# OpenDriveLab/OccNet

Measured on AMD Instinct MI355X. Metric: nuScenes samples/sec (6-cam 900x1600 -> 200x200x16 voxels), higher is better.
Workload: dtype f32 hot path (GEMM operands bf16x3-split, SCA value rows q16 block floating point) + bf16 backbone

## Files before the change

### include/occnet_amd.h

```cpp
#ifndef OCCNET_AMD_H_
#define OCCNET_AMD_H_

#include <stdint.h>

#ifdef __cplusplus
extern "C" {
#endif

#define OCC_OK 0
#define OCC_E_INVALID (-1)
#define OCC_E_LAUNCH (-2)
#define OCC_E_UNSUPPORTED (-3)

int occ_abi_version(void);
const char* occ_last_error(void);
int occ_selftest_fdiv_f32(const float* a, const float* d, float* q, int64_t n, void* stream);


int occ_ms_deform_attn_forward_f32(const float* value, const int64_t* spatial_shapes,
                                   const int64_t* level_start_index, const float* sampling_loc,
                                   const float* attn_weight, float* out, int B, int S, int M, int D,
                                   int L, int Lq, int P, int im2col_step, void* stream);

int occ_ms_deform_attn_backward_f32(const float* value, const int64_t* spatial_shapes,
// ... 113 lines not shown

int occ_sca_prep_forward_f32(const float* proj, int64_t proj_batch_stride, int proj_ld, const int64_t* row_to_query,
                             const float* ref_rb, const int64_t* spatial_shapes, float* loc, float* attn, int B,
                             int64_t R, int M, int L, int P, int Z, void* stream);
int occ_sca_prep_backward_f32(const float* grad_loc, const float* grad_attn, const float* attn,
                              const int64_t* query_to_rows, int Kq, const int64_t* spatial_shapes, float* dproj,
                              int proj_ld, int B, int64_t R, int64_t Q, int M, int L, int P, void* stream);

int occ_rows_gather_sum_f32(const float* x, int64_t x_batch_stride, const int64_t* index, int K, float* out, int B,
                            int64_t rows_out, int64_t rows_in, int F, void* stream);

int64_t occ_linear_wgrad_workspace_bytes(int M, int N, int K);
int occ_linear_wgrad_bf16x3_f32(const float* dy, int64_t lddy, const float* x, int64_t ldx, float* dw, float* db,
                                void* workspace, int64_t workspace_bytes, int M, int N, int K, void* stream);

int64_t occ_conv3d_wgrad_workspace_bytes(int B, int Z, int Y, int X, int Cin);
int occ_conv3d_wgrad_bf16x3_f32(const float* dy_pad, const float* x_pad, float* dw, void* workspace,
                                int64_t workspace_bytes, int B, int Z, int Y, int X, int Cin, void* stream);

int occ_bias_act_nhwc_bf16(void* x, const float* bias, const void* residual, int64_t rows, int C, int relu,
                           void* stream);

int64_t occ_bias_act_bwd_partial_floats(int64_t rows, int C);
int occ_bias_act_bwd_nhwc_bf16(const void* grad_y, const void* y, void* g, float* partial, float* bias_grad,
                               int64_t rows, int C, int relu, void* stream);

int occ_conv_bn_fold_fwd_f32(const float* weight, const float* gamma, const float* beta, const float* rstd,
                             const float* mean_rstd, float* w_folded, void* w_folded_bf16_nhwc, float* bias, int Cout,
                             int Cin, int KH, int KW, void* stream);
int occ_conv_bn_fold_bwd_f32(const void* grad_w_bf16, int64_t stride_o, int64_t stride_i, int64_t stride_h, int64_t stride_w,
                             const float* weight, const float* gamma, const float* rstd, const float* mean_rstd,
                             const float* grad_bias, float* grad_weight, float* grad_gamma, int Cout, int Cin, int KH, int KW,
                             void* stream);

unsigned occ_ln_dropout_hash(unsigned index, unsigned seed_lo, unsigned seed_hi);
int64_t occ_dropout_add_ln_bwd_partial_floats(int64_t rows, int C);
int occ_dropout_add_ln_fwd_f32(const float* x, const float* residual, const float* gamma, const float* beta, float eps,
                               float p_drop, uint64_t seed, float* z, float* y, float* stats, int64_t rows, int C,
                               void* stream);
int occ_dropout_add_ln_bwd_f32(const float* grad_y, const float* z, const float* stats, const float* gamma, float p_drop,
                               uint64_t seed, float* grad_x, float* grad_residual, float* partial, float* grad_gamma_beta,
                               int64_t rows, int C, void* stream);

int occ_value_proj_bf16_f32(int n_segments, const void* const* a, const int64_t* lda, const int64_t* rows,
                            const int64_t* rows_per_group, const int64_t* out_row0,
                            const float* const* group_bias, int bias_groups, const void* weight_packed,
                            float* out, int64_t ldo, int K, int N, int64_t out_group_rows, void* stream);
int occ_value_proj_bf16_f16pairs(int n_segments, const void* const* a, const int64_t* lda, const int64_t* rows,
                            const int64_t* rows_per_group, const int64_t* out_row0,
                            const float* const* group_bias, int bias_groups, const void* weight_packed,
                            void* out, int64_t ldo, int K, int N, int64_t out_group_rows, const float* out_scale,
                            void* stream);
int occ_value_proj_bf16_q16pairs(int n_segments, const void* const* a, const int64_t* lda, const int64_t* rows,
                            const int64_t* rows_per_group, const int64_t* out_row0,
                            const float* const* group_bias, int bias_groups, const void* weight_packed,
                            void* out, int64_t ldo, int K, int N, int64_t out_group_rows, const float* out_scale,
                            void* stream);

int occ_value_range_scale_bf16(int n_segments, const void* const* a, const int64_t* lda, const int64_t* rows, int K,
                               int n_planes, const float* row_l1, const float* bias_max, float* scale_out,
                               uint32_t* work, void* stream);
int occ_value_range_scale_from_amax(const uint32_t* amax8, int n_planes, const float* row_l1, const float* bias_max,
                                    float* scale_out, void* stream);

int occ_value_proj_bf16_planes(int n_segments, const void* const* a, const int64_t* lda, const int64_t* rows,
                               const int64_t* rows_per_group, const int64_t* out_row0,
                               const float* const* group_bias, int bias_groups, const void* weight_packed, void* out,
                               int out_f16, int64_t ldo, int K, int n_planes, int plane_cols, int64_t plane_stride,
                               int64_t out_group_rows, const float* out_scale, void* stream);

int occ_stem_conv7x7_pool_f32_bf16(const float* x, const void* weight_frag, const float* bias, void* out,
                                   int batch, int H, int W, void* stream);
int occ_stem_conv7x7_pool_u8_bf16(const uint8_t* x, const void* weight_frag, const float* bias, void* out,
                                  int batch, int Hs, int Ws, int H, int W, const float* mean,
                                  const float* std, int to_rgb, void* stream);

int occ_bias_relu_maxpool_nhwc_bf16(const void* y, const float* bias, void* out, int batch, int H, int W, int C,
                                    void* stream);

int occ_conv1x1_nhwc_bf16(const void* x, const void* weight, const float* bias, const void* residual,
                          void* out, int batch, int Hin, int Win, int Cin, int Cout, int stride, int relu,
                          int residual_upsample2, void* stream);

int occ_conv3x3_pack_weight_bf16(const float* weight, void* packed, int Cout, int Cin, void* stream);
int occ_conv3x3_nhwc_bf16(const void* x, const void* weight_packed, const float* bias, void* out, int batch,
                          int H, int W, int Cin, int Cout, int stride, int relu, void* stream);
int occ_conv3x3_nhwc_bf16_amax(const void* x, const void* weight_packed, const float* bias, void* out, int batch,
                               int H, int W, int Cin, int Cout, int stride, int relu, uint32_t* amax8, void* stream);

int occ_mfma_pack_b_frag_bf16(const float* weight, void* packed, int N, int K, void* stream);

int occ_bottleneck64_nhwc_bf16(const void* x, const void* w1_frag, const float* b1, const void* w2_frag,
                               const float* b2, const void* w3_frag, const float* b3, void* out, int batch,
                               int H, int W, int Cin, int downsample, void* stream);

#ifdef __cplusplus
}
#endif
#endif
```

### occnet_amd/csrc/conv1x1_nhwc_bf16.hip

```cpp
#include "common.h"

namespace occ {

typedef float f32x16 __attribute__((ext_vector_type(16)));
typedef __bf16 bf16x8 __attribute__((ext_vector_type(8)));


__device__ __forceinline__ float c1_bf16_to_f32(unsigned short h) { return __uint_as_float((unsigned)h << 16); }

template <int NT, int RT>
__global__ __launch_bounds__(256) void conv1x1_nhwc_bf16_kernel(
    const uint4* __restrict__ x, const uint4* __restrict__ w, const float* __restrict__ bias,
    const unsigned short* __restrict__ residual, unsigned short* __restrict__ out, long M, int N, int K,
    int Hin, int Win, int Hout, int Wout, int stride, int relu, int res_up) {
  constexpr int KC = 32, kCLD = KC * 2 + 16, PC = KC / 8;
  constexpr int BM = 32 * RT, BN = 128 * NT, WR = 32 * NT, OLD = BN + 4;
  constexpr int AP = BM * PC / 256;
  constexpr int A_BYTES = BM * kCLD;
  constexpr int STAGE_BYTES = 2 * A_BYTES, OUT_BYTES = 32 * OLD * 4;
  __shared__ __attribute__((aligned(16))) char lds[STAGE_BYTES > OUT_BYTES ? STAGE_BYTES : OUT_BYTES];
  const int tid = threadIdx.x, lane = tid & 63, wave = tid >> 6;
  const int vi = lane & 31, kb = lane >> 5;
  const long m0 = (long)blockIdx.x * BM;
  const int n0 = blockIdx.y * BN;
// ... 57 lines not shown
        af[rt][ks] = *reinterpret_cast<const bf16x8*>(sA + (rt * 32 + vi) * kCLD + ks * 32 + kb * 16); \
    _Pragma("unroll") for (int rt = 0; rt < RT; ++rt) {                                           \
      acc[rt][0] = __builtin_amdgcn_mfma_f32_32x32x16_bf16(af[rt][0], __builtin_bit_cast(bf16x8, wa0_##SW), acc[rt][0], 0, 0, 0); \
      if (NT > 1) acc[rt][NT - 1] = __builtin_amdgcn_mfma_f32_32x32x16_bf16(af[rt][0], __builtin_bit_cast(bf16x8, wa1_##SW), acc[rt][NT - 1], 0, 0, 0); \
    }                                                                                             \
    _Pragma("unroll") for (int rt = 0; rt < RT; ++rt) {                                           \
      acc[rt][0] = __builtin_amdgcn_mfma_f32_32x32x16_bf16(af[rt][1], __builtin_bit_cast(bf16x8, wb0_##SW), acc[rt][0], 0, 0, 0); \
      if (NT > 1) acc[rt][NT - 1] = __builtin_amdgcn_mfma_f32_32x32x16_bf16(af[rt][1], __builtin_bit_cast(bf16x8, wb1_##SW), acc[rt][NT - 1], 0, 0, 0); \
    }                                                                                             \
  }

  const int NCHK = K / KC;
  const int rot = (int)((blockIdx.x * 5u + blockIdx.y * 3u) % (unsigned)NCHK);
#define OCC_C1_K(CI) ((((CI) < NCHK ? (CI) : NCHK - 1) + rot) % NCHK * KC)
  OCC_C1_ISSUE_A(0, OCC_C1_K(0))
  OCC_C1_ISSUE_W(0, OCC_C1_K(0))
  OCC_C1_ISSUE_A(1, OCC_C1_K(1))
  OCC_C1_ISSUE_W(1, OCC_C1_K(1))
  for (int ci = 0; ci < NCHK; ci += 6) {
    OCC_C1_STEP(0, 0, 2, 0, OCC_C1_K(ci + 2))
    if (ci + 1 < NCHK) OCC_C1_STEP(1, 1, 0, 1, OCC_C1_K(ci + 3))
    if (ci + 2 < NCHK) OCC_C1_STEP(0, 2, 1, 0, OCC_C1_K(ci + 4))
    if (ci + 3 < NCHK) OCC_C1_STEP(1, 0, 2, 1, OCC_C1_K(ci + 5))
    if (ci + 4 < NCHK) OCC_C1_STEP(0, 1, 0, 0, OCC_C1_K(ci + 6))
    if (ci + 5 < NCHK) OCC_C1_STEP(1, 2, 1, 1, OCC_C1_K(ci + 7))
  }
#undef OCC_C1_K
#undef OCC_C1_STEP
#undef OCC_C1_ISSUE_A
#undef OCC_C1_ISSUE_W

  const int c = lane * 4;
  const bool col_live = c < BN && n0 + c < N;
  float4 bv = make_float4(0.f, 0.f, 0.f, 0.f);
  if (col_live) bv = *reinterpret_cast<const float4*>(bias + n0 + c);
  float* sO = reinterpret_cast<float*>(lds);
#pragma unroll
  for (int rt = 0; rt < RT; ++rt) {
    __syncthreads();
#pragma unroll
    for (int t = 0; t < NT; ++t)
#pragma unroll
      for (int r = 0; r < 16; ++r)
        sO[((r & 3) + 8 * (r >> 2) + 4 * kb) * OLD + (wave * NT + t) * 32 + vi] = acc[rt][t][r];
    __syncthreads();
    uint2 rv[8];
#pragma unroll
    for (int rr = 0; rr < 8; ++rr) {
      long m = m0 + rt * 32 + wave * 8 + rr;
      if (m >= M) m = M - 1;
      rv[rr] = make_uint2(0u, 0u);
      if (residual != nullptr && col_live) {
        long rrow = m;
        if (res_up) {
          const long hw = (long)Hout * Wout;
          const long n = m / hw, rem = m - n * hw;
          const int yo = (int)(rem / Wout), xo = (int)(rem - (long)yo * Wout);
          rrow = (n * (Hout >> 1) + (yo >> 1)) * (Wout >> 1) + (xo >> 1);
        }
        rv[rr] = *reinterpret_cast<const uint2*>(residual + rrow * N + n0 + c);
      }
    }
#pragma unroll
    for (int rr = 0; rr < 8; ++rr) {
      const int row = wave * 8 + rr;
      const long m = m0 + rt * 32 + row;
      if (m < M && col_live) {
        float4 v = *reinterpret_cast<const float4*>(sO + row * OLD + c);
        v.x += bv.x; v.y += bv.y; v.z += bv.z; v.w += bv.w;
        v.x += c1_bf16_to_f32((unsigned short)(rv[rr].x & 0xffffu));
        v.y += c1_bf16_to_f32((unsigned short)(rv[rr].x >> 16));
        v.z += c1_bf16_to_f32((unsigned short)(rv[rr].y & 0xffffu));
        v.w += c1_bf16_to_f32((unsigned short)(rv[rr].y >> 16));
        if (relu) {
          v.x = fmaxf(v.x, 0.f); v.y = fmaxf(v.y, 0.f); v.z = fmaxf(v.z, 0.f); v.w = fmaxf(v.w, 0.f);
        }
        const uint2 o = make_uint2(pack_bf16x2_rne(v.x, v.y), pack_bf16x2_rne(v.z, v.w));
        *reinterpret_cast<uint2*>(out + m * N + n0 + c) = o;
      }
    }
  }
}

}

extern "C" int occ_conv1x1_nhwc_bf16(const void* x, const void* weight, const float* bias,
                                     const void* residual, void* out, int batch, int Hin, int Win,
                                     int Cin, int Cout, int stride, int relu, int residual_upsample2,
                                     void* stream) {
  using namespace occ;
  OCC_CHECK_ARG(x && weight && bias && out, "conv1x1_nhwc_bf16: null pointer argument");
  OCC_CHECK_ARG(batch > 0 && Hin > 0 && Win > 0 && Cin > 0 && Cout > 0 && stride > 0,
                "conv1x1_nhwc_bf16: bad dimension");
  if (Cin % 32 || Cout % 32) {
    set_error("conv1x1_nhwc_bf16: no kernel for Cin=%d Cout=%d (need Cin %% 32 == 0, Cout %% 32 == 0)", Cin,
              Cout);
    return OCC_E_UNSUPPORTED;
  }
  const int Hout = (Hin - 1) / stride + 1, Wout = (Win - 1) / stride + 1;
  OCC_CHECK_ARG(!residual_upsample2 || (residual && Hout % 2 == 0 && Wout % 2 == 0),
                "conv1x1_nhwc_bf16: an upsampled residual needs even output sizes (exact x2 nearest upsampling)");
  const long M = (long)batch * Hout * Wout;
  hipStream_t st = reinterpret_cast<hipStream_t>(stream);
#define OCC_C1_LAUNCH(NTT, RTT, BNN)                                                                \
  hipLaunchKernelGGL((conv1x1_nhwc_bf16_kernel<NTT, RTT>),                                          \
                     dim3((unsigned)((M + 32 * RTT - 1) / (32 * RTT)), (unsigned)((Cout + BNN - 1) / BNN)), \
                     dim3(256), 0, st, reinterpret_cast<const uint4*>(x),                           \
                     reinterpret_cast<const uint4*>(weight), bias,                                  \
                     reinterpret_cast<const unsigned short*>(residual),                             \
                     reinterpret_cast<unsigned short*>(out), M, Cout, Cin, Hin, Win, Hout, Wout, stride, relu,  \
                     residual_upsample2)
  if (Cout <= 128) OCC_C1_LAUNCH(1, 2, 128); else OCC_C1_LAUNCH(2, 2, 256);
#undef OCC_C1_LAUNCH
  OCC_CHECK_LAUNCH("conv1x1_nhwc_bf16");
  return OCC_OK;
}
```

### occnet_amd/ext.py

```python
import ctypes
import os

import torch

from . import _lib, cache_epoch
from ._lib import OccAmdError, OccAmdUnsupported, f32, i32, i64, ptr, stream_ptr


_TIMING = None
_TIMING_ONLY = None


def kernel_timing(enable=True):
    global _TIMING, _TIMING_ONLY
    _TIMING = {} if enable else None
    _TIMING_ONLY = None
    return _TIMING


def kernel_timing_only(names):
    global _TIMING_ONLY
    _TIMING_ONLY = None if names is None else set(names)


# ... 1284 lines not shown
                                                       i32(H), i32(W), stream_ptr(x.device))
    _note_flops('bb_stem7x7_pool', 2.0 * N * Hc * Wc * 64 * 147)
    _lib.check(rc, "stem_conv7x7_pool")
    return out


def stem_conv7x7_pool_u8(x_u8, weight_frag, bias, mean, std, to_rgb=False, size_divisor=32):
    if not (x_u8.is_cuda and x_u8.dtype == torch.uint8 and x_u8.dim() == 4 and x_u8.shape[-1] == 3
            and x_u8.is_contiguous()):
        raise OccAmdUnsupported("stem_conv7x7_pool_u8: x must be a contiguous (N, H, W, 3) uint8 device tensor")
    _need_cuda_f32("bias", bias)
    if weight_frag.numel() != 64 * 224 or bias.numel() != 64:
        raise OccAmdError("stem_conv7x7_pool_u8: inconsistent shapes")
    N, Hs, Ws, _ = x_u8.shape
    d = int(size_divisor)
    H, W = (Hs + d - 1) // d * d, (Ws + d - 1) // d * d
    Hc, Wc = (H - 1) // 2 + 1, (W - 1) // 2 + 1
    Hp, Wp = (Hc - 1) // 2 + 1, (Wc - 1) // 2 + 1
    out = torch.empty((N, 64, Hp, Wp), dtype=torch.bfloat16, device=x_u8.device, memory_format=torch.channels_last)
    mean_c = (f32 * 3)(*[float(v) for v in mean])
    std_c = (f32 * 3)(*[float(v) for v in std])
    with torch.cuda.device(x_u8.device):
        rc = _lib.lib().occ_stem_conv7x7_pool_u8_bf16(ptr(x_u8), ptr(weight_frag), ptr(bias), ptr(out), i32(N),
                                                      i32(Hs), i32(Ws), i32(H), i32(W), mean_c, std_c,
                                                      i32(1 if to_rgb else 0), stream_ptr(x_u8.device))
    _lib.check(rc, "stem_conv7x7_pool_u8")
    return out, (H, W)


def bias_relu_maxpool_nhwc(y, bias):
    if not (y.is_cuda and y.dtype == torch.bfloat16 and y.dim() == 4
            and y.is_contiguous(memory_format=torch.channels_last)):
        raise OccAmdUnsupported("bias_relu_maxpool_nhwc: y must be a channels_last bfloat16 device tensor")
    _need_cuda_f32("bias", bias)
    N, C, H, W = y.shape
    if bias.numel() != C:
        raise OccAmdError("bias_relu_maxpool_nhwc: bias must have C entries")
    out = torch.empty((N, C, (H - 1) // 2 + 1, (W - 1) // 2 + 1), dtype=torch.bfloat16, device=y.device,
                      memory_format=torch.channels_last)
    with torch.cuda.device(y.device):
        rc = _lib.lib().occ_bias_relu_maxpool_nhwc_bf16(ptr(y), ptr(bias), ptr(out), i32(N), i32(H), i32(W),
                                                        i32(C), stream_ptr(y.device))
    _lib.check(rc, "bias_relu_maxpool_nhwc")
    return out


def conv1x1_pack_weight(weight2d):
    cout, cin = weight2d.shape
    if cin % 32 or cout % 32:
        raise OccAmdUnsupported("conv1x1_pack_weight: Cin and Cout must be multiples of 32")
    return mfma_pack_b_frag(weight2d.float().contiguous())


def conv1x1_nhwc(x, weight_frag, bias, residual=None, relu=False, stride=1, residual_upsample2=False):
    if not (x.is_cuda and x.dtype == torch.bfloat16 and x.dim() == 4
            and x.is_contiguous(memory_format=torch.channels_last)):
        raise OccAmdUnsupported("conv1x1_nhwc: x must be a channels_last bfloat16 device tensor")
    _need_cuda_f32("bias", bias)
    N, Cin, H, W = x.shape
    Cout = bias.numel()
    if not (weight_frag.dtype == torch.int16 and weight_frag.dim() == 1 and weight_frag.is_contiguous()
            and weight_frag.numel() == Cout * Cin):
        raise OccAmdError("conv1x1_nhwc: weight must come from conv1x1_pack_weight (Cout*Cin bf16, fragment order)")
    s = int(stride)
    Ho, Wo = (H - 1) // s + 1, (W - 1) // s + 1
    out = torch.empty((N, Cout, Ho, Wo), dtype=torch.bfloat16, device=x.device,
                      memory_format=torch.channels_last)
    want = (N, Cout, Ho // 2, Wo // 2) if residual_upsample2 else tuple(out.shape)
    if residual_upsample2 and (residual is None or Ho % 2 or Wo % 2):
        raise OccAmdUnsupported("conv1x1_nhwc: an upsampled residual needs even output sizes")
    if residual is not None and not (residual.dtype == torch.bfloat16 and tuple(residual.shape) == want and
                                     residual.is_contiguous(memory_format=torch.channels_last)):
        raise OccAmdUnsupported("conv1x1_nhwc: residual must match the output (channels_last bfloat16)")
    with torch.cuda.device(x.device), _timed('bb_conv1x1'):
        rc = _lib.lib().occ_conv1x1_nhwc_bf16(ptr(x), ptr(weight_frag), ptr(bias), ptr(residual), ptr(out),
                                              i32(N), i32(H), i32(W), i32(Cin), i32(Cout), i32(s),
                                              i32(1 if relu else 0), i32(1 if residual_upsample2 else 0),
                                              stream_ptr(x.device))
    _note_flops('bb_conv1x1', 2.0 * N * Ho * Wo * Cin * Cout)
    _lib.check(rc, "conv1x1_nhwc")
    return out


def mfma_pack_b_frag(weight2d):
    _need_cuda_f32("weight", weight2d)
    if weight2d.dim() != 2:
        raise OccAmdError("mfma_pack_b_frag: expected a (N, K) matrix")
    weight2d = weight2d.contiguous()
    n, k = weight2d.shape
    packed = torch.empty(n * k, dtype=torch.int16, device=weight2d.device)
    with torch.cuda.device(weight2d.device):
        rc = _lib.lib().occ_mfma_pack_b_frag_bf16(ptr(weight2d), ptr(packed), i32(n), i32(k),
                                                  stream_ptr(weight2d.device))
    _lib.check(rc, "mfma_pack_b_frag")
    return packed


def bottleneck64_pack(w1, b1, w2, b2, w3, b3, wds=None, bds=None):
    w1 = w1.float().reshape(w1.shape[0], -1)
    w3 = w3.float().reshape(w3.shape[0], -1)
    if tuple(w2.shape) != (64, 64, 3, 3) or w1.shape[0] != 64 or tuple(w3.shape) != (256, 64):
        raise OccAmdUnsupported("bottleneck64_pack: only 64 mid / 256 output channels")
    ds = wds is not None
    cin = w1.shape[1]
    if (ds and cin != 64) or (not ds and cin != 256):
        raise OccAmdUnsupported("bottleneck64_pack: Cin must be 256 (identity) or 64 (projection)")
    w2m = w2.float().permute(0, 2, 3, 1).reshape(64, 9 * 64)
    b3 = b3.float()
    if ds:
        w3 = torch.cat([w3, wds.float().reshape(256, 64)], dim=1)
        b3 = b3 + bds.float()
    return dict(w1=mfma_pack_b_frag(w1), b1=b1.float().contiguous(), w2=mfma_pack_b_frag(w2m),
                b2=b2.float().contiguous(), w3=mfma_pack_b_frag(w3), b3=b3.contiguous(), cin=cin, ds=ds)


def bottleneck64_nhwc(x, pack):
    if not (x.is_cuda and x.dtype == torch.bfloat16 and x.dim() == 4
            and x.is_contiguous(memory_format=torch.channels_last)):
        raise OccAmdUnsupported("bottleneck64_nhwc: x must be a channels_last bfloat16 device tensor")
    N, Cin, H, W = x.shape
    if Cin != pack['cin']:
        raise OccAmdError("bottleneck64_nhwc: x has %d channels, the pack was built for %d" % (Cin, pack['cin']))
    out = torch.empty((N, 256, H, W), dtype=torch.bfloat16, device=x.device, memory_format=torch.channels_last)
    with torch.cuda.device(x.device), _timed('bb_bottleneck64'):
        rc = _lib.lib().occ_bottleneck64_nhwc_bf16(ptr(x), ptr(pack['w1']), ptr(pack['b1']), ptr(pack['w2']),
                                                   ptr(pack['b2']), ptr(pack['w3']), ptr(pack['b3']), ptr(out),
                                                   i32(N), i32(H), i32(W), i32(Cin), i32(1 if pack['ds'] else 0),
                                                   stream_ptr(x.device))
    _note_flops('bb_bottleneck64', 2.0 * N * H * W * (Cin * 64 + 9 * 64 * 64 + 64 * 256 + (Cin * 256 if pack['ds'] else 0)))
    _lib.check(rc, "bottleneck64_nhwc")
    return out


def conv3x3_pack_weight(weight):
    _need_cuda_f32("weight", weight)
    if weight.dim() != 4 or tuple(weight.shape[2:]) != (3, 3):
        raise OccAmdError("conv3x3_pack_weight: expected a (Cout, Cin, 3, 3) weight")
    cout, cin = weight.shape[:2]
    packed = torch.empty(weight.numel(), dtype=torch.int16, device=weight.device)
    with torch.cuda.device(weight.device):
        rc = _lib.lib().occ_conv3x3_pack_weight_bf16(ptr(weight), ptr(packed), i32(cout), i32(cin),
                                                     stream_ptr(weight.device))
    _lib.check(rc, "conv3x3_pack_weight")
    return packed


def conv3x3_nhwc(x, w_packed, bias, cout, relu=False, stride=1, amax=None):
    if not (x.is_cuda and x.dtype == torch.bfloat16 and x.dim() == 4
            and x.is_contiguous(memory_format=torch.channels_last)):
        raise OccAmdUnsupported("conv3x3_nhwc: x must be a channels_last bfloat16 device tensor")
    _need_cuda_f32("bias", bias)
    N, Cin, H, W = x.shape
    if w_packed.numel() != cout * Cin * 9 or bias.numel() != cout:
        raise OccAmdError("conv3x3_nhwc: inconsistent shapes")
    st = int(stride)
    if st not in (1, 2):
        raise OccAmdUnsupported("conv3x3_nhwc: stride must be 1 or 2")
    if amax is not None and not (amax.is_cuda and amax.dtype == torch.int32 and amax.numel() == 8 and amax.is_contiguous()):
        raise OccAmdError("conv3x3_nhwc: amax must be 8 contiguous int32 device words")
    out = torch.empty((N, cout, (H - 1) // st + 1, (W - 1) // st + 1), dtype=torch.bfloat16, device=x.device,
                      memory_format=torch.channels_last)
    with torch.cuda.device(x.device), _timed('bb_conv3x3'):
        if amax is None:
            rc = _lib.lib().occ_conv3x3_nhwc_bf16(ptr(x), ptr(w_packed), ptr(bias), ptr(out), i32(N), i32(H),
                                                  i32(W), i32(Cin), i32(cout), i32(st), i32(1 if relu else 0),
                                                  stream_ptr(x.device))
# ... 8 lines not shown
```

### occnet_amd/plugin/backbone.py

```python
import os

import torch
import torch.nn as nn
import torch.nn.functional as F

from .. import cache_epoch
from .bricks import BaseModule, ConvModule
from .registry import BACKBONES, NECKS


def conv_bn_folded(x, conv, bn):
    rstd, mean_rstd = _bn_fold_constants(bn)
    s = bn.weight * rstd
    w = conv.weight * s.view(-1, 1, 1, 1)
    b = torch.addcmul(bn.bias, bn.weight, mean_rstd, value=-1.0)
    if conv.bias is not None:
        b = b + conv.bias * s
    return F.conv2d(x, w, b, conv.stride, conv.padding, conv.dilation, conv.groups)


def _bn_fold_constants(bn):
    key = (bn.running_mean._version, bn.running_var._version, bn.running_var.data_ptr(), cache_epoch())
    cached = getattr(bn, '_occ_fold', None)
    if cached is None or cached[0] != key:
# ... 249 lines not shown
                if isinstance(m, nn.modules.batchnorm._BatchNorm):
                    m.eval()
        return self


@NECKS.register_module()
class FPN(BaseModule):

    def __init__(self, in_channels, out_channels, num_outs, start_level=0, end_level=-1,
                 add_extra_convs=False, relu_before_extra_convs=False, no_norm_on_lateral=False,
                 conv_cfg=None, norm_cfg=None, act_cfg=None, upsample_cfg=dict(mode='nearest'),
                 init_cfg=None, **kwargs):
        super().__init__(init_cfg)
        assert isinstance(in_channels, (list, tuple))
        self.in_channels, self.out_channels = in_channels, out_channels
        self.num_ins, self.num_outs = len(in_channels), num_outs
        self.relu_before_extra_convs = relu_before_extra_convs
        self.upsample_cfg = dict(upsample_cfg)
        self.backbone_end_level = self.num_ins if end_level in (-1, self.num_ins - 1) else end_level + 1
        self.start_level = start_level
        if add_extra_convs is True:
            add_extra_convs = 'on_input'
        assert add_extra_convs in (False, 'on_input', 'on_lateral', 'on_output')
        self.add_extra_convs = add_extra_convs
        self.lateral_convs = nn.ModuleList()
        self.fpn_convs = nn.ModuleList()
        for i in range(self.start_level, self.backbone_end_level):
            self.lateral_convs.append(ConvModule(in_channels[i], out_channels, 1, conv_cfg=conv_cfg,
                                                 norm_cfg=None if no_norm_on_lateral else norm_cfg,
                                                 act_cfg=act_cfg, inplace=False))
            self.fpn_convs.append(ConvModule(out_channels, out_channels, 3, padding=1,
                                             conv_cfg=conv_cfg, norm_cfg=norm_cfg, act_cfg=act_cfg,
                                             inplace=False))
        extra_levels = num_outs - self.backbone_end_level + self.start_level
        if self.add_extra_convs and extra_levels >= 1:
            for i in range(extra_levels):
                cin = self.in_channels[self.backbone_end_level - 1] \
                    if (i == 0 and self.add_extra_convs == 'on_input') else out_channels
                self.fpn_convs.append(ConvModule(cin, out_channels, 3, stride=2, padding=1,
                                                 conv_cfg=conv_cfg, norm_cfg=norm_cfg,
                                                 act_cfg=act_cfg, inplace=False))
        for m in self.modules():
            if isinstance(m, nn.Conv2d):
                nn.init.xavier_uniform_(m.weight)
                if m.bias is not None:
                    nn.init.constant_(m.bias, 0)

    @staticmethod
    def _run(cm, x):
        if (_fused_train_ok(x) and not getattr(cm, 'with_norm', False) and not getattr(cm, 'with_activation', False)
                and isinstance(getattr(cm, 'conv', None), nn.Conv2d) and _plain_conv(cm.conv)):
            return conv_bn_act(x, cm.conv, None)
        return cm(x)

    def forward(self, inputs):
        assert len(inputs) == len(self.in_channels)
        laterals = [self._run(conv, inputs[i + self.start_level]) for i, conv in enumerate(self.lateral_convs)]
        n = len(laterals)
        for i in range(n - 1, 0, -1):
            laterals[i - 1] = laterals[i - 1] + F.interpolate(
                laterals[i], size=laterals[i - 1].shape[2:], **self.upsample_cfg)
        outs = [self._run(self.fpn_convs[i], laterals[i]) for i in range(n)]
        if self.num_outs > len(outs):
            if not self.add_extra_convs:
                for _ in range(self.num_outs - n):
                    outs.append(F.max_pool2d(outs[-1], 1, stride=2))
            else:
                if self.add_extra_convs == 'on_input':
                    src = inputs[self.backbone_end_level - 1]
                elif self.add_extra_convs == 'on_lateral':
                    src = laterals[-1]
                else:
                    src = outs[-1]
                outs.append(self._run(self.fpn_convs[n], src))
                for i in range(n + 1, self.num_outs):
                    src = F.relu(outs[-1]) if self.relu_before_extra_convs else outs[-1]
                    outs.append(self._run(self.fpn_convs[i], src))
        return tuple(outs)


class FusedInferenceBackbone(nn.Module):

    def __init__(self, backbone, neck, dtype=torch.bfloat16, fused_ops=False, hip_tail=True,
                 fused_bottleneck=True, prefix_stages=None):
        super().__init__()
        self.prefix_stages = prefix_stages
        self.hip_tail = hip_tail and dtype == torch.bfloat16
        self.use_graph = False
        self._graphs = {}
        from torch.nn.utils.fusion import fuse_conv_bn_weights
        assert not backbone.training or backbone.norm_eval, "folding BN needs eval-mode statistics"
        self.dtype, self.fused_ops = dtype, fused_ops
        self.out_indices = backbone.out_indices
        self._convs = []

        def fold(conv, bn):
            w, b = fuse_conv_bn_weights(conv.weight, conv.bias, bn.running_mean, bn.running_var,
                                        bn.eps, bn.weight, bn.bias)
            return self._add(w, b, conv)

        self.stem = fold(backbone.conv1, backbone.bn1)
        c1, mp = backbone.conv1, backbone.maxpool
        pool_ok = (mp.kernel_size, mp.stride, mp.padding) in ((3, 2, 1), ((3, 3), (2, 2), (1, 1)))
        sw = getattr(self, f'w{self.stem}')
        self._stem_fused = (self.hip_tail and sw.is_cuda and tuple(sw.shape) == (64, 3, 7, 7) and pool_ok
                            and tuple(c1.stride) == (2, 2) and tuple(c1.padding) == (3, 3)
                            and tuple(c1.dilation) == (1, 1) and c1.groups == 1
                            and getattr(mp, 'dilation', 1) in (1, (1, 1)) and not getattr(mp, 'ceil_mode', False))
        if self._stem_fused:
            from .. import ext
            self.register_buffer('stem_frag', ext.stem_pack_weight(sw), persistent=False)
        self.stages = []
        for name in (backbone.res_layers if prefix_stages is None else backbone.res_layers[:prefix_stages]):
            blocks = []
            for blk in getattr(backbone, name):
                ds = None if blk.downsample is None else fold(blk.downsample[0], blk.downsample[1])
                blocks.append((fold(blk.conv1, blk.bn1), fold(blk.conv2, blk.bn2),
                               fold(blk.conv3, blk.bn3), ds))
            self.stages.append(blocks)
        self._bneck = {}
        if fused_bottleneck and self.hip_tail and getattr(self, f'w{self.stem}').is_cuda:
            from .. import ext
            for si, blocks in enumerate(self.stages):
                for bi, (c1, c2, c3, ds) in enumerate(blocks):
                    w1, w2, w3 = (getattr(self, f'w{i}') for i in (c1, c2, c3))
                    ok = (tuple(w2.shape) == (64, 64, 3, 3) and tuple(w3.shape[:2]) == (256, 64)
                          and self._convs[c2][0] == (1, 1) and self._convs[c2][1] == (1, 1)
                          and ((ds is None and w1.shape[1] == 256) or
                               (ds is not None and w1.shape[1] == 64 and self._convs[ds][0] == (1, 1))))
                    if not ok:
                        continue
                    pk = ext.bottleneck64_pack(
                        w1, getattr(self, f'b{c1}'), w2, getattr(self, f'b{c2}'), w3, getattr(self, f'b{c3}'),
                        None if ds is None else getattr(self, f'w{ds}'),
                        None if ds is None else getattr(self, f'b{ds}'))
                    for k in ('w1', 'b1', 'w2', 'b2', 'w3', 'b3'):
                        self.register_buffer(f'k{si}_{bi}_{k}', pk[k], persistent=False)
                    self._bneck[(si, bi)] = (pk['cin'], pk['ds'])
        self.neck = neck
        if neck is None:
            self.laterals, self.fpn = [], []
            return
        self.laterals = [self._add(m.conv.weight, m.conv.bias, m.conv) for m in neck.lateral_convs]
        self.fpn = [self._add(m.conv.weight, m.conv.bias, m.conv) for m in neck.fpn_convs]
        for m in list(neck.lateral_convs) + list(neck.fpn_convs):
            assert not m.with_norm and not m.with_activation, "FPN ConvModules with norm/act not folded"

    def _add(self, w, b, conv):
        w = w.detach().to(self.dtype).contiguous(memory_format=torch.channels_last)
        if b is None:
            b = torch.zeros(w.shape[0], device=w.device)
        b = b.detach().float() if self.hip_tail else b.detach().to(self.dtype)
        idx = len(self._convs)
        self.register_buffer(f'w{idx}', w, persistent=False)
        self.register_buffer(f'b{idx}', b, persistent=False)
        gemm = (self.hip_tail and tuple(conv.kernel_size) == (1, 1) and tuple(conv.padding) == (0, 0)
                and tuple(conv.dilation) == (1, 1) and conv.groups == 1 and conv.stride[0] == conv.stride[1]
                and w.shape[1] % 32 == 0 and w.shape[0] % 32 == 0 and w.is_cuda)
        if gemm:
            from .. import ext
            self.register_buffer(f'm{idx}', ext.conv1x1_pack_weight(w.reshape(w.shape[0], w.shape[1])),
                                 persistent=False)
        c3 = (self.hip_tail and tuple(conv.kernel_size) == (3, 3) and tuple(conv.padding) == (1, 1)
              and tuple(conv.stride) in ((1, 1), (2, 2)) and tuple(conv.dilation) == (1, 1) and conv.groups == 1
              and w.shape[1] % 32 == 0 and w.shape[0] % 128 == 0 and w.is_cuda)
        if c3:
            from .. import ext
            self.register_buffer(f'p{idx}', ext.conv3x3_pack_weight(w.float().contiguous()), persistent=False)
        self._convs.append((conv.stride, conv.padding, conv.dilation, conv.groups))
        self._gemm = getattr(self, '_gemm', {})
        self._gemm[idx] = gemm
        self._c3 = getattr(self, '_c3', {})
        self._c3[idx] = c3
        return idx

    def _conv(self, i, x, relu=False, add=None, amax=None):
        w, b = getattr(self, f'w{i}'), getattr(self, f'b{i}')
        if amax is not None and not (self._c3.get(i) and add is None and not self.fused_ops
                                     and x.is_contiguous(memory_format=torch.channels_last)):
            self._amax_ok = False
        s, p, d, g = self._convs[i]
        if self.fused_ops and add is not None:
            return torch.miopen_convolution_add_relu(x, w, add, 1.0, b.to(w.dtype), s, p, d, g)
        if self.fused_ops and relu:
            return torch.miopen_convolution_relu(x, w, b.to(w.dtype), s, p, d, g)
        if self._gemm.get(i) and x.is_contiguous(memory_format=torch.channels_last) and \
                (add is None or add.is_contiguous(memory_format=torch.channels_last)):
            from .. import ext
            return ext.conv1x1_nhwc(x, getattr(self, f'm{i}'), b, residual=add,
                                    relu=relu or add is not None, stride=s[0])
        if self._c3.get(i) and add is None and x.is_contiguous(memory_format=torch.channels_last):
            from .. import ext
            return ext.conv3x3_nhwc(x, getattr(self, f'p{i}'), b, w.shape[0], relu=relu, stride=s[0],
                                    amax=amax if getattr(self, '_amax_ok', False) else None)
        if self.hip_tail and w.shape[0] % 8 == 0:
            from .. import ext
            y = F.conv2d(x, w, None, s, p, d, g)
            if y.is_contiguous(memory_format=torch.channels_last) and \
                    (add is None or add.is_contiguous(memory_format=torch.channels_last)):
                return ext.bias_act_nhwc_(y, b, residual=add, relu=relu or add is not None)
            y = y + b.to(y.dtype).view(1, -1, 1, 1)
        else:
            y = F.conv2d(x, w, b.to(w.dtype), s, p, d, g)
        if add is not None:
            y = y.add_(add)
        return y.relu_() if (relu or add is not None) else y

    @torch.no_grad()
    def forward(self, x):
        if not getattr(self, 'use_graph', False) or not x.is_cuda:
            return self._forward_eager(x)
        key = (tuple(x.shape), x.dtype, str(x.device))
        st = self._graphs.setdefault(key, dict(calls=0))
        st['calls'] += 1
        if st['calls'] <= 2:
            return self._forward_eager(x)
        if 'graph' not in st:
            st['in'] = x.clone()
            torch.cuda.synchronize(x.device)
            g = torch.cuda.CUDAGraph()
            with torch.cuda.graph(g):
                st['out'] = self._forward_eager(st['in'])
            st['graph'] = g
        st['in'].copy_(x)
        st['graph'].replay()
        return st['out']

    def forward_u8(self, x_u8, mean, std, to_rgb=False, size_divisor=32):
        from .. import ext
        from .._lib import OccAmdUnsupported
        if not getattr(self, '_stem_fused', False):
            raise OccAmdUnsupported("forward_u8 needs the fused stem kernel (bf16 plan, 7x7/s2 stem + 3x3/s2 pool)")
        x, hw = ext.stem_conv7x7_pool_u8(x_u8, self.stem_frag, getattr(self, f'b{self.stem}'), mean, std,
                                         to_rgb=to_rgb, size_divisor=size_divisor)
        return self._forward_stages(x), hw

    def _forward_eager(self, x):
        sw = getattr(self, f'w{self.stem}')
        if getattr(self, '_stem_fused', False) and x.is_cuda and x.dtype == torch.float32 and x.is_contiguous():
            from .. import ext
            x = ext.stem_conv7x7_pool(x, self.stem_frag, getattr(self, f'b{self.stem}'))
            return self._forward_stages(x)
        x = x.to(self.dtype).contiguous(memory_format=torch.channels_last)
        if self.hip_tail and sw.shape[0] % 8 == 0 and x.is_cuda:
            from .. import ext
            s, p, d, g = self._convs[self.stem]
            y = F.conv2d(x, sw, None, s, p, d, g)
            if y.is_contiguous(memory_format=torch.channels_last):
                x = ext.bias_relu_maxpool_nhwc(y, getattr(self, f'b{self.stem}'))
            else:
                x = F.max_pool2d((y + getattr(self, f'b{self.stem}').to(y.dtype).view(1, -1, 1, 1)).relu_(),
                                 kernel_size=3, stride=2, padding=1)
        else:
            x = F.max_pool2d(self._conv(self.stem, x, relu=True), kernel_size=3, stride=2, padding=1)
        return self._forward_stages(x)

    def _run_stage(self, si, x):
        for bi, (c1, c2, c3, ds) in enumerate(self.stages[si]):
            if (si, bi) in self._bneck and x.is_contiguous(memory_format=torch.channels_last):
                from .. import ext
                cin, has_ds = self._bneck[(si, bi)]
                pk = {k: getattr(self, f'k{si}_{bi}_{k}') for k in ('w1', 'b1', 'w2', 'b2', 'w3', 'b3')}
                pk.update(cin=cin, ds=has_ds)
                x = ext.bottleneck64_nhwc(x, pk)
                continue
            identity = x if ds is None else self._conv(ds, x)
            y = self._conv(c2, self._conv(c1, x, relu=True), relu=True)
            x = self._conv(c3, y, add=identity)
        return x

    @torch.no_grad()
    def forward_prefix(self, x):
        from .. import ext
        x = ext.stem_conv7x7_pool(x, self.stem_frag, getattr(self, f'b{self.stem}'))
        for si in range(len(self.stages)):
            x = self._run_stage(si, x)
        return x

    def _forward_stages(self, x):
        feats = []
        for si in range(len(self.stages)):
            x = self._run_stage(si, x)
            if si in self.out_indices:
                feats.append(x)
        nk = self.neck
        inputs = feats
        n = len(self.laterals)
        lat = [None] * n
        nearest = nk.upsample_cfg.get('mode', 'nearest') == 'nearest' and 'scale_factor' not in nk.upsample_cfg
        for i in range(n - 1, -1, -1):
            xin = inputs[i + nk.start_level]
            li = self.laterals[i]
            up = lat[i + 1] if i + 1 < n else None
            if up is not None and nearest and self._gemm.get(li) and xin.shape[2] == 2 * up.shape[2] \
                    and xin.shape[3] == 2 * up.shape[3] and xin.is_contiguous(memory_format=torch.channels_last):
                from .. import ext
                lat[i] = ext.conv1x1_nhwc(xin, getattr(self, f'm{li}'), getattr(self, f'b{li}'), residual=up,
                                          relu=False, residual_upsample2=True)
                continue
            lat[i] = self._conv(li, xin)
            if up is not None:
                lat[i] = lat[i] + F.interpolate(up, size=lat[i].shape[2:], **nk.upsample_cfg)
        amax = None
        self._amax_ok = bool(lat[0].is_cuda and self.dtype == torch.bfloat16)
        if self._amax_ok:
            from .. import ext
            amax = ext.new_absmax_words(lat[0].device)
        outs = [self._conv(self.fpn[i], lat[i], amax=amax) for i in range(n)]
        if nk.num_outs > n:
            if not nk.add_extra_convs:
                for _ in range(nk.num_outs - n):
                    outs.append(F.max_pool2d(outs[-1], 1, stride=2))
            else:
                if nk.add_extra_convs == 'on_input':
                    src = inputs[nk.backbone_end_level - 1]
                elif nk.add_extra_convs == 'on_lateral':
                    src = lat[-1]
                else:
                    src = outs[-1]
                outs.append(self._conv(self.fpn[n], src, amax=amax))
                for i in range(n + 1, nk.num_outs):
                    src = F.relu(outs[-1]) if nk.relu_before_extra_convs else outs[-1]
                    outs.append(self._conv(self.fpn[i], src, amax=amax))
        if self._amax_ok:
            from .. import ext
            for o in outs:
                ext.attach_absmax(o, amax)
        return tuple(outs)
```

Baseline: 184.4.

## Fuse bottleneck downsample conv into conv3 GEMM and add LDS-pipelined conv1x1 kernel

Adds a conv1x1 GEMM kernel that stages tiles through LDS via global_load_lds double buffering, uses swizzled A rows and block-grouped scheduling, and is selected for large problem sizes. A dual mode concatenates the K dimension of conv3 (over y) and the downsample conv (over strided x), so the residual branch is computed in the same accumulator. This avoids writing and re-reading the identity tensor and saves one launch per downsample block. The cost is more kernel variants and a change in rounding, since the residual is no longer rounded to bf16 before the add.

After: 186.2 (median of 6 runs). No clear change (+1.0%).

```diff
diff --git a/include/occnet_amd.h b/include/occnet_amd.h
--- a/include/occnet_amd.h
+++ b/include/occnet_amd.h
@@ -219,6 +219,10 @@
                           void* out, int batch, int Hin, int Win, int Cin, int Cout, int stride, int relu,
                           int residual_upsample2, void* stream);
 
+int occ_conv1x1_dual_nhwc_bf16(const void* y, const void* x, const void* weight, const float* bias, void* out,
+                               int batch, int Hout, int Wout, int Cmid, int Hin, int Win, int Cin, int Cout, int stride,
+                               int relu, void* stream);
+
 int occ_conv3x3_pack_weight_bf16(const float* weight, void* packed, int Cout, int Cin, void* stream);
 int occ_conv3x3_nhwc_bf16(const void* x, const void* weight_packed, const float* bias, void* out, int batch,
                           int H, int W, int Cin, int Cout, int stride, int relu, void* stream);
diff --git a/occnet_amd/csrc/conv1x1_nhwc_bf16.hip b/occnet_amd/csrc/conv1x1_nhwc_bf16.hip
--- a/occnet_amd/csrc/conv1x1_nhwc_bf16.hip
+++ b/occnet_amd/csrc/conv1x1_nhwc_bf16.hip
@@ -163,6 +163,219 @@
   }
 }
 
+typedef __attribute__((address_space(3))) void* c1_lds_ptr_t;
+
+constexpr int kC1ScrPitch = 64 * 4 + 16;
+constexpr int kC1ScrBytes = 32 * kC1ScrPitch;
+
+template <int WM, int WN, int RT>
+struct C1Tile {
+  static constexpr int NW = WM * WN, BM = 32 * RT * WM, BN = 64 * WN;
+  static constexpr int A_BYTES = BM * 128;
+  static constexpr int STAGE = A_BYTES + BN * 128;
+  static constexpr int LDS = 2 * STAGE > NW * kC1ScrBytes ? 2 * STAGE : NW * kC1ScrBytes;
+  static constexpr int AI = BM / (8 * NW), BI = BN / (8 * NW);
+  static_assert(AI >= 1 && BI >= 1 && AI * 8 * NW == BM && BI * 8 * NW == BN, "tile / wave split");
+};
+
+__device__ __forceinline__ long c1_pix(long m, int Hout, int Wout, int Hin, int Win, int stride) {
+  if (stride == 1) return m;
+  const long hw = (long)Hout * Wout;
+  const long n = m / hw, rem = m - n * hw;
+  const int yo = (int)(rem / Wout), xo = (int)(rem - (long)yo * Wout);
+  return (n * Hin + (long)yo * stride) * Win + (long)xo * stride;
+}
+
+template <int WM, int WN, int RT, bool DUAL>
+__global__ __launch_bounds__(64 * WM * WN) void conv1x1_lds_kernel(
+    const uint4* __restrict__ x, const uint4* __restrict__ x2, const uint4* __restrict__ w,
+    const float* __restrict__ bias, const unsigned short* __restrict__ residual, unsigned short* __restrict__ out,
+    long M, int N, int K1, int K2, int Hin, int Win, int stride, int Hin2, int Win2, int stride2, int Hout,
+    int Wout, int relu, int res_up, int mtiles, int ntiles) {
+  using T = C1Tile<WM, WN, RT>;
+  extern __shared__ __attribute__((aligned(16))) char lds[];
+  const int tid = threadIdx.x, lane = tid & 63;
+  const int wave = __builtin_amdgcn_readfirstlane(tid >> 6);
+  const int wm = wave / WN, wn = wave % WN;
+  const int vi = lane & 31, kb = lane >> 5;
+  const int id = (int)blockIdx.x, grp = id / (8 * ntiles), within = id - grp * 8 * ntiles;
+  const int rb = grp * 8 + (within & 7), cb = within >> 3;
+  if (rb >= mtiles) return;
+  const long m0 = (long)rb * T::BM;
+  const int n0 = cb * T::BN;
+  const int NT32 = N / 32, NKT1 = K1 / 64, NKT = NKT1 + (DUAL ? K2 / 64 : 0);
+
+  const uint4* arow[T::AI];
+  const uint4* arow2[DUAL ? T::AI : 1];
+#pragma unroll
+  for (int j = 0; j < T::AI; ++j) {
+    const int r = (j * T::NW + wave) * 8 + (lane >> 3);
+    long m = m0 + r;
+    if (m >= M) m = M - 1;
+    const int piece = (lane & 7) ^ ((r >> 1) & 7);
+    arow[j] = x + c1_pix(m, Hout, Wout, Hin, Win, stride) * (K1 / 8) + piece;
+    if (DUAL) arow2[DUAL ? j : 0] = x2 + c1_pix(m, Hout, Wout, Hin2, Win2, stride2) * (K2 / 8) + piece;
+  }
+  int boff[T::BI];
+#pragma unroll
+  for (int j = 0; j < T::BI; ++j) {
+    const int g = j * T::NW + wave;
+    const int ks = g / (T::BN / 32), nt = min(n0 / 32 + g % (T::BN / 32), NT32 - 1);
+    boff[j] = (ks * NT32 + nt) * 64 + lane;
+  }
+  const int kt_stride = 4 * NT32 * 64;
+
+#define OCC_C1_ISSUE(KT, BUF)                                                                                   \
+  {                                                                                                             \
+    char* sa_ = lds + (BUF) * T::STAGE;                                                                         \
+    char* sb_ = sa_ + T::A_BYTES;                                                                               \
+    _Pragma("unroll") for (int j = 0; j < T::AI; ++j) {                                                         \
+      const uint4* src = (!DUAL || (KT) < NKT1) ? arow[j] + (KT) * 8 : arow2[DUAL ? j : 0] + ((KT) - NKT1) * 8; \
+      __builtin_amdgcn_global_load_lds(src, (c1_lds_ptr_t)(sa_ + (j * T::NW + wave) * 1024), 16, 0, 0);        \
+    }                                                                                                           \
+    _Pragma("unroll") for (int j = 0; j < T::BI; ++j) {                                                         \
+      const uint4* src = w + boff[j] + (KT) * kt_stride;                                                        \
+      __builtin_amdgcn_global_load_lds(src, (c1_lds_ptr_t)(sb_ + (j * T::NW + wave) * 1024), 16, 0, 0);        \
+    }                                                                                                           \
+  }
+
+  f32x16 acc[RT][2];
+#pragma unroll
+  for (int rt = 0; rt < RT; ++rt)
+#pragma unroll
+    for (int t = 0; t < 2; ++t)
+#pragma unroll
+      for (int r = 0; r < 16; ++r) acc[rt][t][r] = 0.f;
+
+  const int arow0 = wm * 32 * RT + vi;
+  const int bfrag0 = (wn * 2) * 1024 + lane * 16;
+  OCC_C1_ISSUE(0, 0)
+  for (int kt = 0; kt < NKT; ++kt) {
+    asm volatile("s_waitcnt vmcnt(0) lgkmcnt(0)\n\ts_barrier" ::: "memory");
+    if (kt + 1 < NKT) OCC_C1_ISSUE(kt + 1, (kt + 1) & 1)
+    const char* sa = lds + (kt & 1) * T::STAGE;
+    const char* sb = sa + T::A_BYTES;
+#pragma unroll
+    for (int ks = 0; ks < 4; ++ks) {
+      bf16x8 bf[2], af[RT];
+#pragma unroll
+      for (int t = 0; t < 2; ++t)
+        bf[t] = *reinterpret_cast<const bf16x8*>(sb + ks * (T::BN / 32) * 1024 + bfrag0 + t * 1024);
+#pragma unroll
+      for (int rt = 0; rt < RT; ++rt) {
+        const int row = arow0 + rt * 32;
+        af[rt] = *reinterpret_cast<const bf16x8*>(sa + row * 128 + (((2 * ks + kb) ^ ((row >> 1) & 7)) << 4));
+      }
+#pragma unroll
+      for (int rt = 0; rt < RT; ++rt)
+#pragma unroll
+        for (int t = 0; t < 2; ++t)
+          acc[rt][t] = __builtin_amdgcn_mfma_f32_32x32x16_bf16(bf[t], af[rt], acc[rt][t], 0, 0, 0);
+    }
+  }
+#undef OCC_C1_ISSUE
+
+  asm volatile("s_waitcnt lgkmcnt(0)\n\ts_barrier" ::: "memory");
+  char* scr = lds + wave * kC1ScrBytes;
+  const int er = lane >> 3, ec = (lane & 7) * 8;
+  const int n = n0 + wn * 64 + ec;
+  const bool col_live = n < N;
+  float4 b0 = make_float4(0.f, 0.f, 0.f, 0.f), b1 = b0;
+  if (col_live) {
+    b0 = *reinterpret_cast<const float4*>(bias + n);
+    b1 = *reinterpret_cast<const float4*>(bias + n + 4);
+  }
+#pragma unroll
+  for (int rt = 0; rt < RT; ++rt) {
+#pragma unroll
+    for (int t = 0; t < 2; ++t)
+#pragma unroll
+      for (int q = 0; q < 4; ++q)
+        *reinterpret_cast<float4*>(scr + vi * kC1ScrPitch + (t * 32 + 8 * q + 4 * kb) * 4) =
+            make_float4(acc[rt][t][4 * q], acc[rt][t][4 * q + 1], acc[rt][t][4 * q + 2], acc[rt][t][4 * q + 3]);
+    asm volatile("s_waitcnt lgkmcnt(0)" ::: "memory");
+    const long mr0 = m0 + wm * 32 * RT + rt * 32 + er;
+    uint4 rv[4];
+#pragma unroll
+    for (int p = 0; p < 4; ++p) {
+      long m = mr0 + p * 8;
+      if (m >= M) m = M - 1;
+      rv[p] = make_uint4(0u, 0u, 0u, 0u);
+      if (residual != nullptr && col_live) {
+        long rrow = m;
+        if (res_up) {
+          const long hw = (long)Hout * Wout;
+          const long nb = m / hw, rem = m - nb * hw;
+          const int yo = (int)(rem / Wout), xo = (int)(rem - (long)yo * Wout);
+          rrow = (nb * (Hout >> 1) + (yo >> 1)) * (Wout >> 1) + (xo >> 1);
+        }
+        rv[p] = *reinterpret_cast<const uint4*>(residual + rrow * N + n);
+      }
+    }
+#pragma unroll
+    for (int p = 0; p < 4; ++p) {
+      const long m = mr0 + p * 8;
+      const char* sp = scr + (p * 8 + er) * kC1ScrPitch + ec * 4;
+      float4 v0 = *reinterpret_cast<const float4*>(sp), v1 = *reinterpret_cast<const float4*>(sp + 16);
+      if (m < M && col_live) {
+        float v[8] = {v0.x + b0.x, v0.y + b0.y, v0.z + b0.z, v0.w + b0.w, v1.x + b1.x, v1.y + b1.y, v1.z + b1.z, v1.w + b1.w};
+        const unsigned rw[4] = {rv[p].x, rv[p].y, rv[p].z, rv[p].w};
+#pragma unroll
+        for (int i = 0; i < 4; ++i) {
+          v[2 * i] += c1_bf16_to_f32((unsigned short)(rw[i] & 0xffffu));
+          v[2 * i + 1] += c1_bf16_to_f32((unsigned short)(rw[i] >> 16));
+        }
+        if (relu) {
+#pragma unroll
+          for (int i = 0; i < 8; ++i) v[i] = fmaxf(v[i], 0.f);
+        }
+        *reinterpret_cast<uint4*>(out + m * N + n) =
+            make_uint4(pack_bf16x2_rne(v[0], v[1]), pack_bf16x2_rne(v[2], v[3]), pack_bf16x2_rne(v[4], v[5]),
+                       pack_bf16x2_rne(v[6], v[7]));
+      }
+    }
+    asm volatile("s_waitcnt lgkmcnt(0)" ::: "memory");
+  }
+}
+
+struct C1Args {
+  const void *x, *x2, *w;
+  const float* bias;
+  const void* residual;
+  void* out;
+  long M;
+  int N, K1, K2, Hin, Win, stride, Hin2, Win2, stride2, Hout, Wout, relu, res_up;
+};
+
+template <int WM, int WN, int RT, bool DUAL>
+static int c1_launch_lds(const C1Args& a, hipStream_t st) {
+  using T = C1Tile<WM, WN, RT>;
+  const int mtiles = (int)((a.M + T::BM - 1) / T::BM), ntiles = (a.N + T::BN - 1) / T::BN;
+  const long blocks = (long)((mtiles + 7) / 8) * 8 * ntiles;
+  const hipError_t e = hipFuncSetAttribute(reinterpret_cast<const void*>(&conv1x1_lds_kernel<WM, WN, RT, DUAL>),
+                                           hipFuncAttributeMaxDynamicSharedMemorySize, T::LDS);
+  if (e != hipSuccess) {
+    set_error("conv1x1_nhwc_bf16: hipFuncSetAttribute failed: %s", hipGetErrorString(e));
+    return OCC_E_LAUNCH;
+  }
+  hipLaunchKernelGGL((conv1x1_lds_kernel<WM, WN, RT, DUAL>), dim3((unsigned)blocks), dim3(64 * T::NW), T::LDS, st,
+                     reinterpret_cast<const uint4*>(a.x), reinterpret_cast<const uint4*>(a.x2),
+                     reinterpret_cast<const uint4*>(a.w), a.bias, reinterpret_cast<const unsigned short*>(a.residual),
+                     reinterpret_cast<unsigned short*>(a.out), a.M, a.N, a.K1, a.K2, a.Hin, a.Win, a.stride, a.Hin2,
+                     a.Win2, a.stride2, a.Hout, a.Wout, a.relu, a.res_up, mtiles, ntiles);
+  OCC_CHECK_LAUNCH("conv1x1_nhwc_bf16");
+  return OCC_OK;
+}
+
+template <bool DUAL>
+static int c1_dispatch(const C1Args& a, hipStream_t st) {
+  auto blocks = [&](long bm, long bn) { return ((a.M + bm - 1) / bm) * ((a.N + bn - 1) / bn); };
+  if (a.N % 256 == 0 && blocks(256, 256) >= 512) return c1_launch_lds<2, 4, 4, DUAL>(a, st);
+  if (blocks(256, 128) >= 512) return c1_launch_lds<4, 2, 2, DUAL>(a, st);
+  if (blocks(128, 128) >= 512) return c1_launch_lds<2, 2, 2, DUAL>(a, st);
+  return c1_launch_lds<2, 2, 1, DUAL>(a, st);
+}
+
 }
 
 extern "C" int occ_conv1x1_nhwc_bf16(const void* x, const void* weight, const float* bias,
@@ -191,8 +404,36 @@
                      reinterpret_cast<const unsigned short*>(residual),                             \
                      reinterpret_cast<unsigned short*>(out), M, Cout, Cin, Hin, Win, Hout, Wout, stride, relu,  \
                      residual_upsample2)
+  const bool big_tiles = (Cout % 256 == 0 && ((M + 255) / 256) * (Cout / 256) >= 512) ||
+                         ((M + 255) / 256) * ((Cout + 127) / 128) >= 512;
+  if (Cin % 64 == 0 && big_tiles) {
+    const C1Args a{x, nullptr, weight, bias, residual, out, M, Cout, Cin, 0, Hin, Win, stride, 1, 1, 1,
+                   Hout, Wout, relu, residual_upsample2};
+    return c1_dispatch<false>(a, st);
+  }
   if (Cout <= 128) OCC_C1_LAUNCH(1, 2, 128); else OCC_C1_LAUNCH(2, 2, 256);
 #undef OCC_C1_LAUNCH
   OCC_CHECK_LAUNCH("conv1x1_nhwc_bf16");
   return OCC_OK;
 }
+
+extern "C" int occ_conv1x1_dual_nhwc_bf16(const void* y, const void* x, const void* weight, const float* bias,
+                                          void* out, int batch, int Hout, int Wout, int Cmid, int Hin, int Win,
+                                          int Cin, int Cout, int stride, int relu, void* stream) {
+  using namespace occ;
+  OCC_CHECK_ARG(y && x && weight && bias && out, "conv1x1_dual_nhwc_bf16: null pointer argument");
+  OCC_CHECK_ARG(batch > 0 && Hout > 0 && Wout > 0 && Cmid > 0 && Hin > 0 && Win > 0 && Cin > 0 && Cout > 0 &&
+                    stride > 0,
+                "conv1x1_dual_nhwc_bf16: bad dimension");
+  OCC_CHECK_ARG((Hin - 1) / stride + 1 == Hout && (Win - 1) / stride + 1 == Wout,
+                "conv1x1_dual_nhwc_bf16: x (%d x %d) at stride %d does not give the %d x %d output", Hin, Win, stride,
+                Hout, Wout);
+  if (Cmid % 64 || Cin % 64 || Cout % 32) {
+    set_error("conv1x1_dual_nhwc_bf16: no kernel for Cmid=%d Cin=%d Cout=%d (need Cmid, Cin %% 64 == 0, Cout %% 32 == 0)",
+              Cmid, Cin, Cout);
+    return OCC_E_UNSUPPORTED;
+  }
+  const C1Args a{y, x, weight, bias, nullptr, out, (long)batch * Hout * Wout, Cout, Cmid, Cin, Hout, Wout, 1,
+                 Hin, Win, stride, Hout, Wout, relu, 0};
+  return c1_dispatch<true>(a, reinterpret_cast<hipStream_t>(stream));
+}
diff --git a/occnet_amd/ext.py b/occnet_amd/ext.py
--- a/occnet_amd/ext.py
+++ b/occnet_amd/ext.py
@@ -1390,6 +1390,31 @@
     return out
 
 
+def conv1x1_dual_nhwc(y, x, weight_frag, bias, stride=1, relu=True):
+    for name, t in (("y", y), ("x", x)):
+        if not (t.is_cuda and t.dtype == torch.bfloat16 and t.dim() == 4
+                and t.is_contiguous(memory_format=torch.channels_last)):
+            raise OccAmdUnsupported(f"conv1x1_dual_nhwc: {name} must be a channels_last bfloat16 device tensor")
+    _need_cuda_f32("bias", bias)
+    N, Cmid, Ho, Wo = y.shape
+    Nx, Cin, H, W = x.shape
+    Cout = bias.numel()
+    s = int(stride)
+    if Nx != N or (H - 1) // s + 1 != Ho or (W - 1) // s + 1 != Wo:
+        raise OccAmdError("conv1x1_dual_nhwc: x at the stride does not give y's spatial size")
+    if not (weight_frag.dtype == torch.int16 and weight_frag.dim() == 1 and weight_frag.is_contiguous()
+            and weight_frag.numel() == Cout * (Cmid + Cin)):
+        raise OccAmdError("conv1x1_dual_nhwc: weight must come from conv1x1_pack_weight of [W3 | Wds]")
+    out = torch.empty((N, Cout, Ho, Wo), dtype=torch.bfloat16, device=y.device, memory_format=torch.channels_last)
+    with torch.cuda.device(y.device), _timed('bb_conv1x1'):
+        rc = _lib.lib().occ_conv1x1_dual_nhwc_bf16(ptr(y), ptr(x), ptr(weight_frag), ptr(bias), ptr(out), i32(N),
+                                                   i32(Ho), i32(Wo), i32(Cmid), i32(H), i32(W), i32(Cin), i32(Cout),
+                                                   i32(s), i32(1 if relu else 0), stream_ptr(y.device))
+    _note_flops('bb_conv1x1', 2.0 * N * Ho * Wo * (Cmid + Cin) * Cout)
+    _lib.check(rc, "conv1x1_dual_nhwc")
+    return out
+
+
 def mfma_pack_b_frag(weight2d):
     _need_cuda_f32("weight", weight2d)
     if weight2d.dim() != 2:
diff --git a/occnet_amd/plugin/backbone.py b/occnet_amd/plugin/backbone.py
--- a/occnet_amd/plugin/backbone.py
+++ b/occnet_amd/plugin/backbone.py
@@ -355,7 +355,7 @@
 class FusedInferenceBackbone(nn.Module):
 
     def __init__(self, backbone, neck, dtype=torch.bfloat16, fused_ops=False, hip_tail=True,
-                 fused_bottleneck=True, prefix_stages=None):
+                 fused_bottleneck=True, prefix_stages=None, fused_downsample=True):
         super().__init__()
         self.prefix_stages = prefix_stages
         self.hip_tail = hip_tail and dtype == torch.bfloat16
@@ -410,6 +410,21 @@
                     for k in ('w1', 'b1', 'w2', 'b2', 'w3', 'b3'):
                         self.register_buffer(f'k{si}_{bi}_{k}', pk[k], persistent=False)
                     self._bneck[(si, bi)] = (pk['cin'], pk['ds'])
+        self._dual = {}
+        if fused_downsample and self.hip_tail:
+            from .. import ext
+            for si, blocks in enumerate(self.stages):
+                for bi, (c1, c2, c3, ds) in enumerate(blocks):
+                    if (si, bi) in self._bneck or ds is None or not (self._gemm.get(c3) and self._gemm.get(ds)):
+                        continue
+                    w3, wds = getattr(self, f'w{c3}'), getattr(self, f'w{ds}')
+                    if self._convs[c3][0] != (1, 1) or w3.shape[1] % 64 or wds.shape[1] % 64:
+                        continue
+                    wcat = torch.cat([w3.reshape(w3.shape[0], -1), wds.reshape(wds.shape[0], -1)], 1)
+                    self.register_buffer(f'd{si}_{bi}_w', ext.conv1x1_pack_weight(wcat), persistent=False)
+                    self.register_buffer(f'd{si}_{bi}_b', getattr(self, f'b{c3}') + getattr(self, f'b{ds}'),
+                                         persistent=False)
+                    self._dual[(si, bi)] = self._convs[ds][0][0]
         self.neck = neck
         if neck is None:
             self.laterals, self.fpn = [], []
@@ -536,6 +551,15 @@
                 pk = {k: getattr(self, f'k{si}_{bi}_{k}') for k in ('w1', 'b1', 'w2', 'b2', 'w3', 'b3')}
                 pk.update(cin=cin, ds=has_ds)
                 x = ext.bottleneck64_nhwc(x, pk)
+                continue
+            if (si, bi) in self._dual and x.is_contiguous(memory_format=torch.channels_last):
+                y = self._conv(c2, self._conv(c1, x, relu=True), relu=True)
+                if y.is_contiguous(memory_format=torch.channels_last):
+                    from .. import ext
+                    x = ext.conv1x1_dual_nhwc(y, x, getattr(self, f'd{si}_{bi}_w'), getattr(self, f'd{si}_{bi}_b'),
+                                              stride=self._dual[(si, bi)], relu=True)
+                    continue
+                x = self._conv(c3, y, add=self._conv(ds, x))
                 continue
             identity = x if ds is None else self._conv(ds, x)
             y = self._conv(c2, self._conv(c1, x, relu=True), relu=True)
```
